# KalistaW/enterprise_warp

Hardware: AMD Instinct MI355X
Metric: lnL evals/sec (whole node), 45-psr CURN batched; % fp64 MFMA peak (higher is better)
Workload: dtype f64

## Files before the change

enterprise_warp_amd/csrc/chol_dd.hip:

```cpp
#include "ewarp_dev.h"

#include <cstdlib>

#pragma clang fp contract(off)

namespace ewh_dev {
namespace {

constexpr int DD_THREADS = 512;

__device__ __forceinline__ dd dd_sub_mul(dd a, dd x, dd y) {
  const double p = x.hi * y.hi;
  const double pe = fma(x.hi, y.hi, -p) + (x.hi * y.lo + x.lo * y.hi);
  const dd s = dd_two_sum(a.hi, -p);
  return dd_fast(s.hi, s.lo + a.lo - pe);
}
__device__ __forceinline__ void dd_acc_sub(double& th, double& tl, dd x, dd y) {
  const double p = x.hi * y.hi;
  const double e = fma(x.hi, y.hi, -p) + fma(x.hi, y.lo, x.lo * y.hi);
  const double s = th - p, bp = s - th;
  tl += ((th - (s - bp)) + (-p - bp)) - e;
  th = s;
}
__device__ __forceinline__ void lds_wave_sync() { asm volatile("s_waitcnt lgkmcnt(0)" ::: "memory"); }
// ... 264 lines not shown
  }
  if (wave == 0) ldet = wave_sum(ldet);
  if (tid == 0) {
    double lnl = J.K[(long long)(b - b_off) * J.kstride] - 0.5 * qv - 0.5 * ldet - 0.5 * lphi;
    if (!ok || J.fail) lnl = -INFINITY;
    out_units[(long long)p_ * B + b] = lnl;
  }
  __syncthreads();
}

template <int PW, bool RSOLVE = true>
__global__ __launch_bounds__(DD_THREADS) void chol_dd_kernel(const CholJob* __restrict__ jobs, int B, long long u0,
                                                             int b_off, const double* __restrict__ theta, int ldth,
                                                             double* __restrict__ out_units,
                                                             double* __restrict__ scratch, long long scr_per_wg,
                                                             const int* __restrict__ list,
                                                             const int* __restrict__ count, int dbg) {
  extern __shared__ __attribute__((aligned(16))) double2 dd_smem[];
  const int cnt = list ? *count : (int)gridDim.x;
  EWH_DCHECK(!list || cnt >= 0, "chol_dd list count");
  for (int i = blockIdx.x; i < cnt; i += gridDim.x) {
    const long long u = list ? (long long)list[i] : u0 + i;
    chol_ddb_unit<PW, RSOLVE>(jobs, B, u, b_off, theta + (long long)(u % B) * ldth, out_units, scratch, scr_per_wg,
                              dd_smem, dbg);
  }
}

constexpr double VERIFY_FRAC = 0.0625;
__global__ __launch_bounds__(256) void verify_units_kernel(const double* __restrict__ a, const double* __restrict__ b,
                                                           long long u0, long long n, double frac,
                                                           int* __restrict__ list, int* __restrict__ count,
                                                           unsigned long long* __restrict__ total) {
  const long long i = (long long)blockIdx.x * 256 + threadIdx.x;
  if (total && i == 0) atomicAdd(total + 1, (unsigned long long)n);
  if (i >= n) return;
  const long long u = u0 + i;
  const double x = a[u], y = b[u];
  const bool fx = x - x == 0.0, fy = y - y == 0.0;
  const bool bad = frac < 0.0 || !fx || !fy || fabs(x - y) > frac * (1e-6 + 1e-10 * fabs(x));
// ... 5 lines not shown
  }
}

__global__ void count_units_kernel(unsigned long long* __restrict__ total, long long n) {
  if (threadIdx.x == 0) {
    atomicAdd(total, (unsigned long long)n);
    atomicAdd(total + 1, (unsigned long long)n);
  }
}

constexpr int DD_PW_WIDE = 8;
constexpr int DD_LD_PW16 = 512;

template <int PW>
void launch_dd(const UnitSpan& s, long long u0, double* scr, long long scr_per_wg, unsigned grid, const int* list,
               const int* count, int ld, bool r05a) {
  int dbg = 0;
#ifdef EWH_DEV
  if (const char* e = getenv("EWARP_DD_SKIP")) dbg = atoi(e);
#endif
  if (r05a)
    hipLaunchKernelGGL(HIP_KERNEL_NAME(chol_dd_kernel<PW, false>), dim3(grid), dim3(DD_THREADS), dd_lds<PW>(ld), s.st,
                       s.jobs, s.B, u0, s.b_off, s.theta, s.ldth, s.units, scr, scr_per_wg, list, count, dbg);
  else
    hipLaunchKernelGGL(HIP_KERNEL_NAME(chol_dd_kernel<PW, true>), dim3(grid), dim3(DD_THREADS), dd_lds<PW>(ld), s.st,
                       s.jobs, s.B, u0, s.b_off, s.theta, s.ldth, s.units, scr, scr_per_wg, list, count, dbg);
}

int launch_dd_any(const UnitSpan& s, long long u0, double* scr, long long scr_per_wg, unsigned grid, const int* list,
                  const int* count, int ld, bool r05a) {
  if (ld <= DD_LD_PW16)
    launch_dd<16>(s, u0, scr, scr_per_wg, grid, list, count, ld, r05a);
  else
    launch_dd<DD_PW_WIDE>(s, u0, scr, scr_per_wg, grid, list, count, ld, r05a);
  const hipError_t e = hipGetLastError();
  return e == hipSuccess ? 0 : set_err(EWH_E_HIP, std::string("chol_dd_kernel: ") + hipGetErrorString(e));
}

}

int set_dd_attributes() {
  if (hipFuncSetAttribute((const void*)chol_dd_kernel<16, true>, hipFuncAttributeMaxDynamicSharedMemorySize,
                          (int)dd_lds<16>(DD_LD_PW16)) != hipSuccess ||
      hipFuncSetAttribute((const void*)chol_dd_kernel<DD_PW_WIDE, true>, hipFuncAttributeMaxDynamicSharedMemorySize,
                          (int)dd_lds<DD_PW_WIDE>(WIDE_LD_MAX)) != hipSuccess ||
// ... 25 lines not shown
  return e == hipSuccess ? 0 : set_err(EWH_E_HIP, std::string("verify_units_kernel: ") + hipGetErrorString(e));
}

long long dd_scratch_per_wg(int ld) { return 2LL * ld * ld; }

int launch_chol_dd(const UnitSpan& s, double* scr, long long scr_per_wg, long long cap, int ld, bool r05a) {
  for (long long o = 0; o < s.n; o += cap) {
    const int rc = launch_dd_any(s, s.u0 + o, scr, scr_per_wg, (unsigned)std::min(cap, s.n - o), nullptr, nullptr, ld,
                                 r05a);
    if (rc) return rc;
  }
  return 0;
}

int launch_chol_dd_list(const UnitSpan& s, double* scr, long long scr_per_wg, long long cap, const int* list,
                        const int* count, int ld, bool r05a) {
  return launch_dd_any(s, 0LL, scr, scr_per_wg, (unsigned)cap, list, count, ld, r05a);
}

}
```

enterprise_warp_amd/csrc/chol_partial.hip:

```cpp
#include "ewarp_dev.h"

namespace ewh_dev {
namespace {

template <int NB, int KEEP>
int launch_partial(const UnitSpan& s, double* keep_out, int keep_bs) {
  if constexpr (partial_in_registers(NB, KEEP) && NB - KEEP >= Split<NB>::H) {
    hipLaunchKernelGGL(HIP_KERNEL_NAME(chol_mfma_kernel<NB, default_waves(NB), PANEL_2L, false, KEEP>),
                       dim3((unsigned)s.n), dim3(64), 0, s.st, s.jobs, s.B, s.u0, s.b_off, s.theta, s.ldth, s.units,
                       keep_out, 0, keep_bs, UnitDec{});
    return 0;
  } else {
    return set_err(EWH_E_UNSUPPORTED, "common: reduced basis too narrow for the kept common block");
  }
}

}

int launch_partial_nb(int nb, int keep, const UnitSpan& s, double* keep_out, int keep_bs) {
  if (!partial_in_registers(nb, keep))
    return set_err(EWH_E_UNSUPPORTED, "common: no register kernel for this reduced width and kept size");
#define EWH_PARTK(NBV, KV) \
  case KV: return launch_partial<NBV, KV>(s, keep_out, keep_bs);
#define EWH_PART(NBV)   \
  case NBV:             \
// ... 26 lines not shown
```

enterprise_warp_amd/csrc/ewarp_chol_small.h:

```cpp
#pragma once
#include "ewarp_dev.h"

namespace ewh_dev {
namespace {

template <int NB, int ALG = PANEL_2L, bool STAMP = false, int W = default_waves(NB), bool FULL = false, int DEAD = -1,
          bool IMG = false, bool PL = false>
void launch_chol_mfma(const UnitSpan& s) {
  constexpr bool PLB = PL && pl_built(NB, DEAD, IMG);
  hipLaunchKernelGGL(HIP_KERNEL_NAME(chol_mfma_kernel<NB, W, ALG, STAMP, 0, FULL, DEAD, IMG, PLB>), dim3((unsigned)s.n),
                     dim3(64), 0, s.st, s.jobs, s.B, s.u0, s.b_off, s.theta, s.ldth, s.units, nullptr, 0, 0,
                     PLB ? unit_dec_make(s.u0, s.B) : UnitDec{});
}

template <int NB, bool STAMP = false, bool IMG = false, bool PL = false>
void launch_chol_front(int dead, const UnitSpan& s) {
  constexpr int W = default_waves(NB);
  switch (front_inst(NB, dead)) {
    case 3: launch_chol_mfma<NB, PANEL_2L, STAMP, W, false, 3, IMG, PL>(s); break;
    case 2: launch_chol_mfma<NB, PANEL_2L, STAMP, W, false, 2, IMG, PL>(s); break;
    case 1: launch_chol_mfma<NB, PANEL_2L, STAMP, W, false, NB == 6 ? -1 : 1, IMG, PL>(s); break;
    default: launch_chol_mfma<NB, PANEL_2L, STAMP, W, false, -1, IMG, PL>(s); break;
  }
}

template <int NB, bool STAMP = false, bool PL = false>
void launch_chol_images(int dead, bool img, const UnitSpan& s) {
// ... 9 lines not shown
```

enterprise_warp_amd/csrc/ewarp_ctx.h:

```cpp
#pragma once

#include "ewarp_launch.h"
#include "ewarp_mem.h"

#include <utility>

namespace ewh_host {

using namespace ewh_dev;
using namespace ewh_mem;

constexpr size_t LDS_MAX = 160 * 1024;

struct PsrHost {
  int n_toa = 0, m = 0, nlead = 0, ld = 0, nb = 0, n_epoch = 0;
  int max_epoch = 0;
  int fx_m = 0, fx_ld = 0, fx_nb = 0;
  int ncommon = 0, nloc = 0, gstart = 0;
  int gstart_v = 0;
  PsrDev dev{};
  int* d_colptr = nullptr;
  DSpec* d_spec = nullptr;
  int* d_fx_colptr = nullptr;
  DSpec* d_fx_spec = nullptr;
// ... 51 lines not shown
    Buf<double> d_dR, d_dZ, d_dcol, d_dcollo;
    long long s_stride = 0;
    int chunk = 0;
    void release() {
      for (auto* b : {&d_w, &d_beta, &d_s, &d_G, &d_Kb, &d_fac, &d_rho, &d_Glo, &d_dR, &d_dZ, &d_dcol, &d_dcollo})
        b->release();
      chunk = 0;
    }
  } var;
  Buf<double> d_bigscr;
  long long scr_budget = 0;
  Buf<double> d_widescr;
  Buf<double> d_ddscr;
  Buf<double> d_units2;
  Buf<int> d_ddlist;
  unsigned long long* d_ddstat = nullptr;
  int n_delay_psr = 0;
  bool cond_all = false;
  struct CondChunk {
    Buf<double> d_theta, d_z, d_x, d_coef, d_V, d_Y;
    Buf<int> d_status, d_grp;
    void release() {
      for (auto* b : {&d_theta, &d_z, &d_x, &d_coef, &d_V, &d_Y}) b->release();
      d_status.release();
      d_grp.release();
    }
  } cond;
  struct JointChunk {
    Buf<double> d_L, d_S, d_rhs, d_xc, d_z;
    Buf<int> d_pstat, d_sfail, d_cstart, d_grp;
    void release() {
// ... 104 lines not shown
```

enterprise_warp_amd/csrc/ewarp_dev.h:

```cpp
#pragma once
#include <hip/hip_runtime.h>

#include <algorithm>
#include <cmath>
#include <cstdint>
#include <cstring>
#include <string>
#include <type_traits>
#include <vector>

#include "ewarp_hip.h"
#include "ewarp_route.h"
#include "ewarp_spec.h"

namespace ewh_dev {

int set_err(int code, const std::string& msg);

#define EWH_HIP(expr)                                                          \
  do {                                                                         \
    hipError_t e_ = (expr);                                                    \
    if (e_ != hipSuccess)                                                      \
      return ::ewh_dev::set_err(EWH_E_HIP, std::string(#expr) + ": " + hipGetErrorString(e_)); \
  } while (0)
// ... 223 lines not shown
  const int* rep = nullptr;
  const int* ulist = nullptr;
  int nu = 0;
  const struct URec* urec = nullptr;
  const int* urep = nullptr;
  int ntidx = 0;
  int tidx[16] = {};
  const double* mats_lo = nullptr;
  const double* mats_rev = nullptr;
  const double* img = nullptr;
  const double* img_front = nullptr;
  const PlRec* pl = nullptr;
  int pl_ne = 0;
};

struct UnitSpan {
  const CholJob* jobs; int B; long long u0, n; int b_off;
  const double* theta; int ldth; double* units; hipStream_t st;
};

struct URec {
  static constexpr int NE = 3;
  DSpec e[NE];
  int ne, pad_[3];
};
static_assert(PL_NE == URec::NE, "a compact record (ewarp_spec.h) holds what a staged record holds");
constexpr int STAGE_THETA_MAX = 512;
constexpr int TIDX_MAX = 16;

template <int NB>
__global__ __launch_bounds__(256) void contract_mfma_kernel(PsrDev P, const double* __restrict__ w,
                                                            const double* __restrict__ beta,
                                                            const double* __restrict__ s,
// ... 775 lines not shown
      if constexpr (!LASTR) {
        const double rs = rsqrt_nr(dv);
        hook.on_scale(r, rs);
        static_for<bb + 1, NB>([&](auto JJ) { blk(JJ)[r] *= rs; });
      }
    });
  }
  }
}

#ifdef EWH_DEV
constexpr int STAMP_UNITS = 4096, STAMP_N = 24;
static __device__ long long g_stamps[STAMP_UNITS * STAMP_N];
#endif

template <int NB, int W, int ALG = PANEL_2L, bool STAMP = false, int KEEP = 0, bool FULL = false, int DEAD = -1,
          bool IMG = false, bool PL = false>
__global__ __launch_bounds__(64) __attribute__((amdgpu_waves_per_eu(W, W)))
void chol_mfma_kernel(const CholJob* __restrict__ jobs, int B, long long u0, int b_off,
                      const double* __restrict__ theta, int ldth, double* __restrict__ out_units,
                      double* __restrict__ keep_out, int keep_b0, int keep_bs, UnitDec ud) {
#ifdef EWH_DEV
  long long stp[STAMP_N];
#define EWH_STAMP(I)                                            \
  if constexpr (STAMP) {                                        \
    __builtin_amdgcn_sched_barrier(0);                          \
    stp[(I)] = (long long)__builtin_amdgcn_s_memtime();         \
    __builtin_amdgcn_sched_barrier(0);                          \
  }
#else
  static_assert(!STAMP, "phase stamps exist only in the dev library");
#define EWH_STAMP(I)
#endif
  EWH_STAMP(0)
  constexpr int LD = 16 * NB;
  using S = Split<NB, FULL>;
// ... 165 lines not shown
        double ph = 0.0;
        if (dedup) {
          ph = phs[J.rep[a]];
        } else {
          for (int e = J.col_ptr[a]; e < J.col_ptr[a + 1]; ++e) ph += spec_phi_body(J.spec[e], th);
        }
        pi = 1.0 / ph;
        ldet.add(ph);
      }
      phinv[wa] = pi;
    }
  }
  __syncthreads();
  EWH_STAMP(1)

  auto load_block = [&](auto BI, auto BJ, v4d& v) {
    constexpr int bi = decltype(BI)::value, bj = decltype(BJ)::value;
    if constexpr (IMG) {
      image_block(BI, BJ, v);
    } else {
      static_for<0, 4>([&](auto R) {
        constexpr int r = decltype(R)::value;
        if constexpr (FRONT) {
          v[r] = front_elem<NB, DEAD, bi, bj, r>(Af, q, c, s);
        } else {
          v[r] = A[(long long)(16 * bi + q + 4 * r) * LD + 16 * bj + c];
        }
      });
    }
    if constexpr (bi == bj) {
      const double pd = phinv[16 * bi + c];
      static_for<0, 4>([&](auto R) {
        constexpr int r = decltype(R)::value;
        v[r] += (q + 4 * r == c) ? pd : 0.0;
      });
    }
  };

  bool ok = true;
  constexpr bool SKIPPAD = KEEP == 0 && !FRONT;
  const int klast = SKIPPAD ? __builtin_amdgcn_readfirstlane(J.mreal - 16 * (NB - 1)) : 16;
  constexpr int D0 = FRONT ? DEAD : 0;
  constexpr bool PACK1 = NB != 8;

  v4d U1[S::n1 > 0 ? S::n1 : 1];
  static_for<0, H>([&](auto BI) {
    constexpr int bi = decltype(BI)::value;
    static_for<bi, NB>([&](auto BJ) {
      constexpr int bj = decltype(BJ)::value;
      if constexpr (bi == 0) {
        U1[S::i1(0, bj)] = pre[bj];
        if constexpr (bj == 0) {
          const double pd = phinv[c];
          static_for<0, 4>([&](auto R) {
            constexpr int r = decltype(R)::value;
            U1[S::i1(0, 0)][r] += (q + 4 * r == c) ? pd : 0.0;
          });
        }
      } else {
        load_block(BI, BJ, U1[S::i1(bi, bj)]);
      }
    });
  });
  static_for<0, H>([&](auto BBc) {
    constexpr int bb = decltype(BBc)::value;
    panel_ldl_row<NB, ALG, KEEP == 0, PACK1, DEAD, BLKLD>(
        BBc, [&](auto JJ) -> v4d& { return U1[S::i1(bb, decltype(JJ)::value)]; }, q, c, ldet, ok, NoHook{}, klast, s);
    EWH_STAMP(2 + 2 * bb)
    static_for<bb + 1, H>([&](auto II) {
      constexpr int i = decltype(II)::value;
      static_for<i, NB>([&](auto JJ) {
        constexpr int j = decltype(JJ)::value;
        syrk_update<bb == 0 ? D0 : 0>(U1[S::i1(i, j)], U1[S::i1(bb, i)], U1[S::i1(bb, j)]);
// ... 50 lines not shown
          const double v = U2[S::i2(i, j)][r];
          if (i != j || row <= col) {
            ko[row * KD + col] = v;
            ko[col * KD + row] = v;
          }
        });
      });
    });
  }
  const double ldet_v = wave_sum(ldet.value());
  const bool ok_all = __all(ok);
  if (lane == 0) {
    double lnl = J.K[(long long)(b - b_off) * J.kstride] - 0.5 * qv - 0.5 * ldet_v;
    if (!ok_all || J.fail) lnl = -INFINITY;
    out_units[(long long)p * B + b] = lnl;
  }
#ifdef EWH_DEV
  if constexpr (STAMP) {
    EWH_STAMP(3 + 2 * NB)
    if (lane == 0 && blockIdx.x < STAMP_UNITS) {
      long long* o = g_stamps + (long long)blockIdx.x * STAMP_N;
      for (int i = 0; i < 4 + 2 * NB && i < STAMP_N - 2; ++i) o[i] = stp[i];
      o[STAMP_N - 2] = __builtin_amdgcn_s_getreg(4 | (31 << 11));
      o[STAMP_N - 1] = __builtin_amdgcn_s_getreg(20 | (31 << 11));
    }
  }
#endif
#undef EWH_STAMP
}
constexpr int WIDE_LD_MAX = 16 * WIDE_NB_MAX;
// ... 114 lines not shown
int launch_chol_small(int mode, int nb, int dead, bool img, bool pl, const UnitSpan& s);
void launch_chol_small_pl(int nb, int dead, bool img, bool stamp, const UnitSpan& s);
int launch_chol_big_nb(int nb, const UnitSpan& s, double* scr, long long cap);
constexpr int LAT_NB_MAX = 8;
constexpr unsigned long long LAT_STALL_BITS = 0x7ff4dead057a1100ull;
int launch_chol_lat(int nb, int dead, const CholJob* jobs, int B, int P, const double* theta, int ldth, double* units,
                    double* host_units, hipStream_t st, bool stamp = false, int var = 0);
long long wide_scratch_per_wg(int nb, int keep);
long long dd_scratch_per_wg(int ld);
int launch_chol_dd(const UnitSpan& s, double* scr, long long scr_per_wg, long long cap, int ld, bool r05a = false);
int set_dd_attributes();
int launch_verify_units(const double* a, const double* b, long long u0, long long n, int* list, int* count,
                        unsigned long long* total, hipStream_t st, bool all = false);
int launch_count_units(unsigned long long* total, long long n, hipStream_t st);
int launch_chol_dd_list(const UnitSpan& s, double* scr, long long scr_per_wg, long long cap, const int* list,
                        const int* count, int ld, bool r05a = false);
int launch_chol_wide(const UnitSpan& s, double* scr, long long scr_per_wg, long long cap, int keep, double* keep_out,
                     int keep_b0, int keep_bs, int rev = 0, double* units_rev = nullptr, bool pair = true);
int launch_partial_nb(int nb, int keep, const UnitSpan& s, double* keep_out, int keep_bs);
int set_contract_attributes();
int launch_contract_wide(int nb, const PsrDev& P, const double* w, const double* beta, const double* s,
                         const double* fac, double* G, int nb_samples, hipStream_t st, double* Glo);
bool variant_built(int mode);

}
```

enterprise_warp_amd/csrc/ewarp_hip.hip:

```cpp
#include "ewarp_ctx.h"

#include <atomic>
#include <chrono>
#include <map>
#include <mutex>

namespace ewh_dev {

thread_local std::string g_err;

int set_err(int code, const std::string& msg) {
  g_err = msg;
  return code;
}

__global__ __launch_bounds__(256) void chol_lds_kernel(const CholJob* __restrict__ jobs, int B,
                                                       long long u0, int b_off,
                                                       const double* __restrict__ theta, int ldth,
                                                       double* __restrict__ out_units) {
  extern __shared__ __attribute__((aligned(16))) double sm[];
  __shared__ double red[4];
  const long long u = u0 + blockIdx.x;
  const int p = (int)(u / B), b = (int)(u % B);
  const CholJob J = jobs[p];
// ... 30 lines not shown
    for (int i = k + 1 + wave; i < ma; i += 4) {
      const double ci = col[i];
      const int base = i * (i + 1) / 2;
      for (int j = k + 1 + lane; j <= i; j += 64) L[base + j] = fma(-ci, col[j], L[base + j]);
    }
    __syncthreads();
  }
  const double qv = L[(ma - 1) * ma / 2 + ma - 1];
  if (threadIdx.x == 0) {
    double lnl = J.K[(long long)(b - b_off) * J.kstride] - 0.5 * qv - 0.5 * ldet.value() - 0.5 * lphi_sum;
    if (!ok || J.fail) lnl = -INFINITY;
    out_units[(long long)p * B + b] = lnl;
  }
}

__global__ void reduce_units_kernel(const double* __restrict__ units, int P, int B, double* __restrict__ out) {
  const int b = blockIdx.x * blockDim.x + threadIdx.x;
  if (b >= B) return;
  double s = 0.0;
  for (int p = 0; p < P; ++p) s += units[(long long)p * B + b];
  out[b] = s;
}

__global__ __launch_bounds__(256) void expand_theta_kernel(const double* __restrict__ stage,
                                                           const int* __restrict__ seg, int nseg, int np,
                                                           double* __restrict__ theta) {
  const int* rec = seg + 5 * blockIdx.x;
  const int r0 = rec[0], nr = rec[1] - rec[0], nc = rec[2];
  const int* cols = seg + 5 * nseg + rec[3];
  const double* src = stage + rec[4];
  for (int idx = threadIdx.x; idx < nr * nc; idx += 256) {
    const int r = idx / nc, j = idx - r * nc;
    theta[(long long)(r0 + r) * np + cols[j]] = src[idx];
  }
}

// ... 65 lines not shown
}

size_t n_units(const DevCtx* h, int B) { return (size_t)(h->P + (h->corr ? 1 : 0)) * B; }

int launch_wide(DevCtx* h, int nb, int keep, const UnitSpan& s, double* keep_out, int rev = 0,
                double* units_rev = nullptr) {
  if (nb > WIDE_NB_MAX) return set_err(EWH_E_UNSUPPORTED, "basis wider than 1023 columns");
  const long long per = wide_scratch_per_wg(nb, keep);
  const long long cap = scratch_slots(h, h->d_widescr, per, 4096);
  if (cap <= 0 || (units_rev && cap < 2)) return EWH_E_NOMEM;
  return launch_chol_wide(s, h->d_widescr.p, per, cap, keep, keep_out, 0, s.B, rev, units_rev, !h->plan.wide_r05a);
}

int ensure_dd_lists(DevCtx* h, const UnitSpan& s, bool list) {
  if (!h->d_ddstat) {
    if (const int rc = dalloc(h, &h->d_ddstat, 2)) return rc;
    EWH_HIP(hipMemsetAsync(h->d_ddstat, 0, 2 * sizeof(unsigned long long), s.st));
  }
  return list ? h->d_ddlist.reserve(n_units(h, s.B) + 1, h->hook) : 0;
}

int launch_dd_path(DevCtx* h, int nb, const UnitSpan& s) {
  const long long per = dd_scratch_per_wg(16 * nb);
  const long long cap = scratch_slots(h, h->d_ddscr, per, 1024);
  if (cap <= 0) return EWH_E_NOMEM;
  int rc;
  if ((rc = ensure_dd_lists(h, s, false))) return rc;
  if (h->plan.all_dd) {
    if ((rc = launch_count_units(h->d_ddstat, s.n, s.st))) return rc;
    return launch_chol_dd(s, h->d_ddscr.p, per, cap, 16 * nb, h->plan.wide_r05a);
  }
  if ((rc = h->d_units2.reserve(n_units(h, s.B), h->hook)) || (rc = ensure_dd_lists(h, s, true))) return rc;
  const bool fuse = !h->plan.wide_r05a && 2 * s.n <= 8LL * h->n_cu;
  if (!fuse) {
    UnitSpan r = s;
    r.units = h->d_units2.p;
    if ((rc = launch_wide(h, nb, 0, s, nullptr, 0)) || (rc = launch_wide(h, nb, 0, r, nullptr, 1))) return rc;
  } else if ((rc = launch_wide(h, nb, 0, s, nullptr, 0, h->d_units2.p))) {
    return rc;
  }
  int *count = h->d_ddlist.p, *list = count + 1;
  EWH_HIP(hipMemsetAsync(count, 0, sizeof(int), s.st));
  if ((rc = launch_verify_units(s.units, h->d_units2.p, s.u0, s.n, list, count, h->d_ddstat, s.st))) return rc;
  return launch_chol_dd_list(s, h->d_ddscr.p, per, std::min<long long>(cap, s.n), list, count, 16 * nb,
                             h->plan.wide_r05a);
}

struct Segment { Source src; int p0, nb, mreal; UnitSpan span; };

template <class F>
int for_segments(const DevCtx* h, const UnitSpan& all, F&& body) {
  const long long B = all.B, u_end = all.u0 + all.n;
  for (long long u = all.u0, end; u < u_end; u = end) {
    const int p0 = (int)(u / B);
    const PsrHost& ps = h->psr[p0];
    const bool run = h->white_fixed && ps.delay.n_delay == 0;
    Segment g{run ? Source::FixedRun : h->white_fixed ? Source::FixedDelay : Source::Varying, p0,
              run ? ps.fx_nb : ps.nb, run ? ps.fx_m : ps.m, all};
    int p1 = p0 + 1;
    for (; run && p1 * B < u_end && h->psr[p1].fx_nb == g.nb && h->psr[p1].delay.n_delay == 0; ++p1)
      g.mreal = std::max(g.mreal, h->psr[p1].fx_m);
    end = std::min(u_end, run ? p1 * B : std::min((p0 + 1) * B, u + h->var.chunk));
    g.span.jobs = run ? h->d_jobs_fixed : h->d_jobs_var;
    g.span.u0 = u;
    g.span.n = end - u;
    g.span.b_off = run ? 0 : (int)(u - p0 * B);
    if (const int rc = body(g)) return rc;
  }
  return 0;
}

int refine_failed(DevCtx* h, const Segment& g) {
  const UnitSpan& s = g.span;
  const long long per = dd_scratch_per_wg(16 * g.nb);
  const long long cap = scratch_slots(h, h->d_ddscr, per, 1024);
  if (cap <= 0) return EWH_E_NOMEM;
  int rc;
  if ((rc = ensure_dd_lists(h, s, true))) return rc;
  int *count = h->d_ddlist.p, *list = count + 1;
  EWH_HIP(hipMemsetAsync(count, 0, sizeof(int), s.st));
  if ((rc = launch_verify_units(s.units, s.units, s.u0, s.n, list, count, h->d_ddstat, s.st,
                                refine_lists_all(g.src, g.nb, h->plan))))
    return rc;
  if (g.src == Source::Varying) {
    const PsrHost& ps = h->psr[g.p0];
    launch_gram_dd_units(ps.dev, ps.nb, (unsigned)std::min<long long>(s.n, 64), ps.d_Tlo, h->var.d_w.p, h->var.d_beta.p,
                         list, count, s.B, s.b_off, h->var.d_G.p, h->var.d_Glo.p, s.st);
    if (ps.delay.n_delay > 0)
      launch_delay_scatter(ps.ld, (int)s.n, h->var.d_dcol.p, h->var.d_dcollo.p, h->var.d_G.p, h->var.d_Glo.p, s.st);
    EWH_HIP(hipGetLastError());
  }
  return launch_chol_dd_list(s, h->d_ddscr.p, per, std::min<long long>(cap, s.n), list, count, 16 * g.nb, false);
}

int partial_units(DevCtx* h, int nb, const UnitSpan& s, double* keep_out) {
  if (partial_route_for(h->plan, nb, h->keep) == PartialRoute::Register)
    return launch_partial_nb(nb, h->keep, s, keep_out, s.B);
  return launch_wide(h, nb, h->keep, s, keep_out);
}

#ifdef EWH_DEV
std::atomic<long long> g_prologue_launches[2] = {{0}, {0}};
#endif

int launch_register(DevCtx* h, const Segment& g) {
  const UnitSpan& s = g.span;
  const int dead = h->osmode ? 0 : front_dead(16 * g.nb, g.mreal);
// ... 200 lines not shown
  }
  if ((rc = corr_partial(h, theta_dev, B, 0, h->P, h->d_units.p, h->d_keep.p, st))) return rc;
  if (overlap) EWH_HIP(hipStreamWaitEvent(st, h->ev_join, 0));
  return corr_finish(h, theta_dev, B, h->d_keep.p, h->d_units.p, st, overlap);
}

int ctx_units(DevCtx* h, const double* theta_dev, int B, int64_t u_begin, int64_t u_end, double* out_dev,
              hipStream_t st, bool reduce) {
  const long long U = (long long)h->P * B;
  u_begin = std::max<int64_t>(0, u_begin);
  u_end = std::min<int64_t>(U, u_end);
  EWH_HIP(hipSetDevice(h->device));
  int rc;
  if ((rc = reserve_units(h, B))) return rc;
  const int rows = h->P + (h->corr ? 1 : 0);
  EWH_HIP(hipMemsetAsync(h->d_units.p, 0, sizeof(double) * (size_t)rows * B, st));
  StreamScope on_st(h, st);
  if (h->corr) {
    if (u_begin != 0 || u_end != U)
      return set_err(EWH_E_UNSUPPORTED, "correlated common process: pass the whole batch (shard samples, not units)");
    if ((rc = lnl_correlated(h, theta_dev, B, st))) return rc;
  } else {
    if ((rc = reserve_var_scratch(h, B))) return rc;
    const UnitSpan all{nullptr, B, u_begin, u_end - u_begin, 0, theta_dev, h->n_param, h->d_units.p, st};
    rc = for_segments(h, all, [&](const Segment& g) {
      const PsrHost& ps = h->psr[g.p0];
      const UnitSpan& s = g.span;
      int rc = 0;
      if (g.src == Source::Varying && (rc = run_white(h, g.p0, s.theta, s.ldth, s.b_off, (int)s.n))) return rc;
      if (g.src != Source::FixedRun && ps.delay.n_delay > 0 &&
          (rc = run_delay(h, g.p0, s.theta, s.ldth, s.b_off, (int)s.n)))
        return rc;
      if ((rc = dispatch_chol(h, g))) return rc;
      if (refine_after(g.src, g.nb, ps.dev.n_bgroup > 0, h->plan, h->corr, h->osmode)) rc = refine_failed(h, g);
      return rc;
    });
    if (rc) return rc;
  }
  if (reduce)
    hipLaunchKernelGGL(reduce_units_kernel, dim3((B + 255) / 256), dim3(256), 0, st, h->d_units.p, rows, B, out_dev);
  EWH_HIP(hipGetLastError());
  h->last_B = B;
  return 0;
}

int reserve_io(DevCtx* h, int B) {
  const size_t nth = (size_t)B * std::max(1, h->n_param);
  const int rc = h->d_theta.reserve(nth + B, h->hook);
  h->d_out = rc ? nullptr : h->d_theta.p + nth;
  return rc;
}

std::vector<std::pair<long long, long long>> unit_ranges(const std::vector<double>& cost, int B, int world) {
  const int P = (int)cost.size();
  std::vector<std::pair<long long, long long>> out;
// ... 424 lines not shown
    }
    if ((rc = corr_partial(h, h->d_theta.p, B, p0, p1, h->d_units.p, h->d_keep.p, h->stream))) return rc;
    if (i > 0) {
      EWH_HIP(hipMemcpyPeerAsync(h0->d_keep.p + (size_t)p0 * B * kd2, h0->device, h->d_keep.p + (size_t)p0 * B * kd2,
                                 h->device, sizeof(double) * (size_t)(p1 - p0) * B * kd2, h->stream));
      EWH_HIP(hipMemcpyPeerAsync(h0->d_units.p + (size_t)p0 * B, h0->device, h->d_units.p + (size_t)p0 * B, h->device,
                                 sizeof(double) * (size_t)(p1 - p0) * B, h->stream));
    }
  }
  for (int i = 1; i < nd; ++i) {
    EWH_HIP(hipSetDevice(H->ctx[i]->device));
    EWH_HIP(hipStreamSynchronize(H->ctx[i]->stream));
  }
  EWH_HIP(hipSetDevice(h0->device));
  if ((rc = corr_finish(h0, h0->d_theta.p, B, h0->d_keep.p, h0->d_units.p, h0->stream))) return rc;
  hipLaunchKernelGGL(reduce_units_kernel, dim3((B + 255) / 256), dim3(256), 0, h0->stream, h0->d_units.p, P + 1, B,
                     h0->d_out);
  EWH_HIP(hipGetLastError());
  EWH_HIP(hipMemcpyAsync(H->h_out.p, h0->d_out, sizeof(double) * B, hipMemcpyDeviceToHost, h0->stream));
  EWH_HIP(hipStreamSynchronize(h0->stream));
  std::memcpy(out_host, H->h_out.p, sizeof(double) * B);
  H->last_split.assign(1, {0, (long long)P * B});
  H->last_B = B;
  h0->last_B = B;
  return 0;
}

constexpr uint64_t LAT_SENTINEL = 0x7ff4dead0ebeef01ull;
constexpr int LAT_B_MAX = 24;

int lnl_batch_single(ewh_handle* H, DevCtx* h, int B, double* out_host) {
  int rc;
// ... 394 lines not shown
  EWH_HIP(hipGetLastError());
  return 0;
}

int ewh_corr_finish_device(ewh_handle* H, const double* theta_dev, int32_t B, const double* keep_dev,
                           const double* local_dev, double* out_dev, void* stream) {
  if (!H || !H->corr || !theta_dev || !keep_dev || !local_dev || !out_dev || B <= 0)
    return set_err(EWH_E_INVALID, "bad arguments (needs a correlated-common-process handle)");
  DevCtx* h = H->ctx[0];
  hipStream_t st = (hipStream_t)stream;
  EWH_HIP(hipSetDevice(h->device));
  int rc;
  if ((rc = reserve_units(h, B))) return rc;
  EWH_HIP(hipMemcpyAsync(h->d_units.p, local_dev, sizeof(double) * (size_t)H->P * B, hipMemcpyDeviceToDevice, st));
  if ((rc = corr_finish(h, theta_dev, B, keep_dev, h->d_units.p, st))) return rc;
  hipLaunchKernelGGL(reduce_units_kernel, dim3((B + 255) / 256), dim3(256), 0, st, h->d_units.p, H->P + 1, B, out_dev);
  EWH_HIP(hipGetLastError());
  H->last_split.assign(1, {0, (long long)H->P * B});
  H->last_B = B;
  h->last_B = B;
  return 0;
}

int ewh_optstat(ewh_handle* H, const double* theta_host, int32_t B, const double* phihat_host, double* rho_host,
                double* sig_host, double* os_host, double* os_sig_host) {
  if (!H) return set_err(EWH_E_INVALID, "bad arguments");
  return ctx_optstat(H->ctx[0], theta_host, B, phihat_host, rho_host, sig_host, os_host, os_sig_host);
}

int ewh_cond_dims(const ewh_handle* H, int64_t* n_coef, int64_t* n_toa_total) {
  if (!H) return set_err(EWH_E_INVALID, "bad handle");
// ... 190 lines not shown
```

enterprise_warp_amd/csrc/ewarp_plan.h:

```cpp
#pragma once

namespace ewh_dev {

struct KernelPlan {
  bool in_range = true;
  bool valid = true;
  bool variant = false;
  bool lat = true;
  bool lat_stamps = false;
  int lat_variant = 0;
  bool lds_only = false;
  bool all_wide = false;
  bool all_dd = false;
  bool refine = true;
  bool wide_r05a = false;
  bool contract2 = true;
  bool rsep = true;
  int contract2_waves = 0;
  bool epoch_multi = true;
  bool fixed_gram_dd = true;
  bool stage_spectra = true;
  bool compact_spectra = true;
  bool minv_reg = true;
  bool corr_right = true;
  bool corr_fuse_diag = true;
  bool corr_fused = true;
  bool corr_pairs = true;
  bool corr_rowupdate_r1 = false;
  bool corr_diag_lds = false;
  bool corr_one_tile = false;
// ... 12 lines not shown
  switch (mode) {
    case 0: p.lat = true; dev_only = false; break;
    case 1:
      p.lds_only = true; p.refine = false;
      p.corr_fused = false; p.corr_rowupdate_r1 = true; p.corr_diag_lds = true;
      dev_only = false;
      break;
    case 2: dev_only = false; break;
    case 7:
      p.contract2 = false; p.fixed_gram_dd = false; p.minv_reg = false;
      p.corr_fused = false; p.corr_diag_lds = true; p.corr_trailing = true;
      dev_only = false;
      break;
    case 27: p.all_wide = true; p.refine = false; dev_only = false; break;
    case 29: p.all_dd = true; dev_only = false; break;
    case 14: p.compact_spectra = false; p.variant = true; break;
    case 15: p.contract2_waves = 4; p.variant = true; break;
    case 16: p.contract2_waves = 8; p.variant = true; break;
    case 17: case 21: case 26: p.variant = true; break;
    case 19: p.stage_spectra = false; p.variant = true; break;
    case 22: p.lat = true; p.lat_stamps = true; p.variant = true; break;
    case 23: p.lat = true; p.lat_variant = 3; p.variant = true; break;
    case 24: p.lat = true; p.lat_variant = 1; p.variant = true; break;
    case 25: p.lat = true; p.lat_variant = 2; p.variant = true; break;
    case 28: p.corr_pairs = false; p.corr_one_tile = true; p.variant = true; break;
    case 30: p.rsep = false; p.contract2_waves = 30; p.variant = true; break;
    case 31: p.corr_pairs = false; p.variant = true; break;
    case 32: p.corr_pair_unpiped = true; p.variant = true; break;
    case 33: p.corr_fuse_diag = false; break;
    case 34: p.wide_r05a = true; break;
    case 35: p.contract2_waves = 35; break;
    case 36: p.rsep = false; break;
    case 37: p.epoch_multi = false; break;
    case 38: p.rsep = false; p.contract2_waves = 38; break;
    case 39: p.rsep = false; p.contract2_waves = 39; break;
    default: p.valid = false; break;
  }
  if (dev_only && !dev_lib) p.valid = false;
  return p;
}

constexpr bool same_plan(const KernelPlan& a, const KernelPlan& b) {
  return a.in_range == b.in_range && a.valid == b.valid && a.variant == b.variant && a.lat == b.lat &&
         a.lat_stamps == b.lat_stamps && a.lat_variant == b.lat_variant && a.lds_only == b.lds_only && a.all_wide == b.all_wide &&
         a.all_dd == b.all_dd && a.refine == b.refine && a.wide_r05a == b.wide_r05a && a.contract2 == b.contract2 &&
         a.rsep == b.rsep && a.contract2_waves == b.contract2_waves && a.epoch_multi == b.epoch_multi &&
         a.fixed_gram_dd == b.fixed_gram_dd && a.stage_spectra == b.stage_spectra && a.compact_spectra == b.compact_spectra &&
         a.minv_reg == b.minv_reg &&
         a.corr_right == b.corr_right && a.corr_fuse_diag == b.corr_fuse_diag && a.corr_fused == b.corr_fused &&
         a.corr_pairs == b.corr_pairs && a.corr_rowupdate_r1 == b.corr_rowupdate_r1 &&
         a.corr_diag_lds == b.corr_diag_lds && a.corr_one_tile == b.corr_one_tile &&
         a.corr_pair_unpiped == b.corr_pair_unpiped && a.corr_trailing == b.corr_trailing;
}

constexpr KernelPlan batched_default_plan() {
  KernelPlan p;
  p.lat = false;
  p.corr_right = false;
  return p;
}

static_assert(same_plan(plan_for(0, false), KernelPlan{}) && same_plan(plan_for(0, true), KernelPlan{}),
              "mode 0 is the default plan");
static_assert(same_plan(plan_for(2, false), batched_default_plan()),
              "mode 2 leaves the latency path and (with every non-default mode) the right-looking schedule, no more");
static_assert(!plan_for(-1, true).in_range && !plan_for(KERNEL_MODE_MAX + 1, true).in_range &&
                  plan_for(3, true).in_range && plan_for(KERNEL_MODE_MAX, false).in_range,
              "the range of mode numbers");
static_assert(plan_for(14, true).valid && !plan_for(14, true).compact_spectra && plan_for(14, true).stage_spectra &&
                  plan_for(19, true).compact_spectra && !plan_for(14, false).valid,
              "mode 14 turns off the fixed-form prologue alone, in the dev library");
static_assert(!plan_for(-1, true).valid && !plan_for(3, true).valid && !plan_for(18, true).valid &&
                  !plan_for(20, true).valid && !plan_for(KERNEL_MODE_MAX + 1, true).valid,
              "a mode outside the lists is invalid");
static_assert(plan_for(33, true).valid && !plan_for(33, false).valid && !plan_for(15, false).valid &&
                  !plan_for(39, false).valid,
              "a dev-only mode is invalid in the product library");
static_assert(plan_for(1, false).valid && plan_for(7, false).valid && plan_for(27, false).valid &&
                  plan_for(29, false).valid,
              "the product modes");

}
```

enterprise_warp_amd/csrc/ewarp_route.h:

```cpp
#pragma once
#include "ewarp_plan.h"

namespace ewh_dev {

constexpr int MFMA_NB_MAX = 9;
constexpr int BIG_NB_MAX = 16;
constexpr int WIDE_NB_MAX = 64;

constexpr int PARTIAL_KEEP_MAX = 4;
constexpr bool partial_in_registers(int nb, int keep) {
  return nb <= MFMA_NB_MAX && keep >= 1 && keep <= PARTIAL_KEEP_MAX && nb - keep >= (nb == 8 ? 3 : nb / 2) &&
         !(nb == 7 && keep >= 3);
}

enum class Route {
  Register,
  Big,
  Lds,
  Wide,
  DdVerify,
  DdAll,
  Unsupported,
};
enum class PartialRoute { Register, Wide };
// ... 21 lines not shown
constexpr PartialRoute partial_route_for(const KernelPlan& plan, int nb, int keep) {
  return partial_in_registers(nb, keep) && !plan.all_wide ? PartialRoute::Register : PartialRoute::Wide;
}

constexpr bool refine_after(Source src, int nb, bool bgroups, const KernelPlan& plan, bool corr, bool osmode) {
  if (corr || osmode || !plan.refine) return false;
  switch (src) {
    case Source::FixedRun: return !dd_path(plan, corr, osmode, nb, true);
    case Source::FixedDelay: return nb <= BIG_NB_MAX;
    default: return !bgroups;
  }
}

constexpr bool refine_lists_all(Source src, int nb, const KernelPlan& plan) {
  return plan.all_dd && src == Source::Varying && nb <= BIG_NB_MAX;
}

namespace route_check {

constexpr Route R = Route::Register, G = Route::Big, L = Route::Lds, W = Route::Wide, V = Route::DdVerify,
                A = Route::DdAll, U = Route::Unsupported;

constexpr bool row(int mode, bool fixed, Route r1, Route r9, Route r10, Route r16, Route r17, Route r64, Route r65) {
  for (int dev = 0; dev < 2; ++dev) {
    const KernelPlan p = plan_for(mode, dev == 1);
    if (route_for(p, false, false, 1, fixed) != r1 || route_for(p, false, false, 9, fixed) != r9 ||
        route_for(p, false, false, 10, fixed) != r10 || route_for(p, false, false, 16, fixed) != r16 ||
        route_for(p, false, false, 17, fixed) != r17 || route_for(p, false, false, 64, fixed) != r64 ||
        route_for(p, false, false, 65, fixed) != r65)
      return false;
// ... 52 lines not shown
  return true;
}
static_assert(same_as_old(0, 9), "routes and refine conditions as before, modes 0..9");
static_assert(same_as_old(10, 19), "routes and refine conditions as before, modes 10..19");
static_assert(same_as_old(20, 29), "routes and refine conditions as before, modes 20..29");
static_assert(same_as_old(30, KERNEL_MODE_MAX), "routes and refine conditions as before, modes 30..");

constexpr bool no_refine(int mode) {
  for (int nb = 1; nb <= 65; ++nb)
    for (int src = 0; src < 3; ++src)
      if (refine_after((Source)src, nb, false, plan_for(mode, false), false, false)) return false;
  return true;
}
static_assert(no_refine(1) && no_refine(27), "the cross-check modes compare the fp64 kernels as such");

constexpr bool partial_as_old() {
  for (int mode = 0; mode <= KERNEL_MODE_MAX; ++mode)
    for (int nb = 1; nb <= 17; ++nb)
      for (int keep = 0; keep <= 5; ++keep) {
        const KernelPlan p = plan_for(mode, true);
        if ((partial_route_for(p, nb, keep) == PartialRoute::Register) !=
            (partial_in_registers(nb, keep) && !p.all_wide))
          return false;
      }
  return true;
}
static_assert(partial_as_old(), "the partial route: registers where the kernel exists, unless all_wide");

}
}
// ... 1 lines not shown
```

Baseline: 1.222 million.

## Fuse failure listing into Cholesky kernel and self-reset DD counters

The register-route Cholesky kernel now appends non-finite units to the refine list and updates the stats counters itself, so fixed-run segments skip the separate verify kernel. The DD refine kernel resets its count with a last-block ticket, which removes the per-segment memsets, and the units buffer memset is skipped for full-range non-correlated evaluations. The refine grid shrinks to the CU count when listing is fused, and the reduce kernel is rewritten to stage rows through LDS. This adds global atomics and relies on every unit being written, plus a new mode 13 that keeps the old path.

```diff
diff --git a/enterprise_warp_amd/csrc/chol_dd.hip b/enterprise_warp_amd/csrc/chol_dd.hip
--- a/enterprise_warp_amd/csrc/chol_dd.hip
+++ b/enterprise_warp_amd/csrc/chol_dd.hip
@@ -302,15 +302,24 @@
                                                              int b_off, const double* __restrict__ theta, int ldth,
                                                              double* __restrict__ out_units,
                                                              double* __restrict__ scratch, long long scr_per_wg,
-                                                             const int* __restrict__ list,
-                                                             const int* __restrict__ count, int dbg) {
+                                                             const int* __restrict__ list, int* count, int dbg) {
   extern __shared__ __attribute__((aligned(16))) double2 dd_smem[];
-  const int cnt = list ? *count : (int)gridDim.x;
+  const int cnt = list ? __hip_atomic_load(count, __ATOMIC_RELAXED, __HIP_MEMORY_SCOPE_AGENT) : (int)gridDim.x;
   EWH_DCHECK(!list || cnt >= 0, "chol_dd list count");
   for (int i = blockIdx.x; i < cnt; i += gridDim.x) {
     const long long u = list ? (long long)list[i] : u0 + i;
     chol_ddb_unit<PW, RSOLVE>(jobs, B, u, b_off, theta + (long long)(u % B) * ldth, out_units, scratch, scr_per_wg,
                               dd_smem, dbg);
+  }
+  if (list && threadIdx.x == 0) {
+    __threadfence();
+    const int ticket = atomicAdd(count + 1, 1);
+    EWH_DCHECK(ticket >= 0 && ticket < (int)gridDim.x, "chol_dd done-ticket within the grid");
+    if (ticket == (int)gridDim.x - 1) {
+      __threadfence();
+      __hip_atomic_store(count, 0, __ATOMIC_RELAXED, __HIP_MEMORY_SCOPE_AGENT);
+      __hip_atomic_store(count + 1, 0, __ATOMIC_RELAXED, __HIP_MEMORY_SCOPE_AGENT);
+    }
   }
 }
 
@@ -346,7 +355,7 @@
 
 template <int PW>
 void launch_dd(const UnitSpan& s, long long u0, double* scr, long long scr_per_wg, unsigned grid, const int* list,
-               const int* count, int ld, bool r05a) {
+               int* count, int ld, bool r05a) {
   int dbg = 0;
 #ifdef EWH_DEV
   if (const char* e = getenv("EWARP_DD_SKIP")) dbg = atoi(e);
@@ -360,7 +369,7 @@
 }
 
 int launch_dd_any(const UnitSpan& s, long long u0, double* scr, long long scr_per_wg, unsigned grid, const int* list,
-                  const int* count, int ld, bool r05a) {
+                  int* count, int ld, bool r05a) {
   if (ld <= DD_LD_PW16)
     launch_dd<16>(s, u0, scr, scr_per_wg, grid, list, count, ld, r05a);
   else
@@ -416,7 +425,7 @@
 }
 
 int launch_chol_dd_list(const UnitSpan& s, double* scr, long long scr_per_wg, long long cap, const int* list,
-                        const int* count, int ld, bool r05a) {
+                        int* count, int ld, bool r05a) {
   return launch_dd_any(s, 0LL, scr, scr_per_wg, (unsigned)cap, list, count, ld, r05a);
 }
 
diff --git a/enterprise_warp_amd/csrc/chol_partial.hip b/enterprise_warp_amd/csrc/chol_partial.hip
--- a/enterprise_warp_amd/csrc/chol_partial.hip
+++ b/enterprise_warp_amd/csrc/chol_partial.hip
@@ -8,7 +8,7 @@
   if constexpr (partial_in_registers(NB, KEEP) && NB - KEEP >= Split<NB>::H) {
     hipLaunchKernelGGL(HIP_KERNEL_NAME(chol_mfma_kernel<NB, default_waves(NB), PANEL_2L, false, KEEP>),
                        dim3((unsigned)s.n), dim3(64), 0, s.st, s.jobs, s.B, s.u0, s.b_off, s.theta, s.ldth, s.units,
-                       keep_out, 0, keep_bs, UnitDec{});
+                       keep_out, 0, keep_bs, UnitDec{}, FailList{});
     return 0;
   } else {
     return set_err(EWH_E_UNSUPPORTED, "common: reduced basis too narrow for the kept common block");
diff --git a/enterprise_warp_amd/csrc/ewarp_chol_small.h b/enterprise_warp_amd/csrc/ewarp_chol_small.h
--- a/enterprise_warp_amd/csrc/ewarp_chol_small.h
+++ b/enterprise_warp_amd/csrc/ewarp_chol_small.h
@@ -10,7 +10,7 @@
   constexpr bool PLB = PL && pl_built(NB, DEAD, IMG);
   hipLaunchKernelGGL(HIP_KERNEL_NAME(chol_mfma_kernel<NB, W, ALG, STAMP, 0, FULL, DEAD, IMG, PLB>), dim3((unsigned)s.n),
                      dim3(64), 0, s.st, s.jobs, s.B, s.u0, s.b_off, s.theta, s.ldth, s.units, nullptr, 0, 0,
-                     PLB ? unit_dec_make(s.u0, s.B) : UnitDec{});
+                     PLB ? unit_dec_make(s.u0, s.B) : UnitDec{}, s.fails);
 }
 
 template <int NB, bool STAMP = false, bool IMG = false, bool PL = false>
diff --git a/enterprise_warp_amd/csrc/ewarp_ctx.h b/enterprise_warp_amd/csrc/ewarp_ctx.h
--- a/enterprise_warp_amd/csrc/ewarp_ctx.h
+++ b/enterprise_warp_amd/csrc/ewarp_ctx.h
@@ -89,7 +89,9 @@
   Buf<double> d_ddscr;
   Buf<double> d_units2;
   Buf<int> d_ddlist;
+  static constexpr int DDSTAT_WORDS = 3;
   unsigned long long* d_ddstat = nullptr;
+  int* dd_count() const { return reinterpret_cast<int*>(d_ddstat + 2); }
   int n_delay_psr = 0;
   bool cond_all = false;
   struct CondChunk {
diff --git a/enterprise_warp_amd/csrc/ewarp_dev.h b/enterprise_warp_amd/csrc/ewarp_dev.h
--- a/enterprise_warp_amd/csrc/ewarp_dev.h
+++ b/enterprise_warp_amd/csrc/ewarp_dev.h
@@ -261,9 +261,15 @@
   int pl_ne = 0;
 };
 
+struct FailList {
+  int* count = nullptr;
+  int* list = nullptr;
+  unsigned long long* stat = nullptr;
+};
 struct UnitSpan {
   const CholJob* jobs; int B; long long u0, n; int b_off;
   const double* theta; int ldth; double* units; hipStream_t st;
+  FailList fails = {};
 };
 
 struct URec {
@@ -1069,12 +1075,14 @@
 static __device__ long long g_stamps[STAMP_UNITS * STAMP_N];
 #endif
 
+constexpr bool diag_by_selectors(int nb, int keep, int alg, bool full, int dead, bool img, bool pl) { return keep == 0; }
+
 template <int NB, int W, int ALG = PANEL_2L, bool STAMP = false, int KEEP = 0, bool FULL = false, int DEAD = -1,
           bool IMG = false, bool PL = false>
 __global__ __launch_bounds__(64) __attribute__((amdgpu_waves_per_eu(W, W)))
 void chol_mfma_kernel(const CholJob* __restrict__ jobs, int B, long long u0, int b_off,
                       const double* __restrict__ theta, int ldth, double* __restrict__ out_units,
-                      double* __restrict__ keep_out, int keep_b0, int keep_bs, UnitDec ud) {
+                      double* __restrict__ keep_out, int keep_b0, int keep_bs, UnitDec ud, FailList fl) {
 #ifdef EWH_DEV
   long long stp[STAMP_N];
 #define EWH_STAMP(I)                                            \
@@ -1270,6 +1278,20 @@
   __syncthreads();
   EWH_STAMP(1)
 
+  constexpr bool DIAGSEL = diag_by_selectors(NB, KEEP, ALG, FULL, DEAD, IMG, PL);
+  [[maybe_unused]] double dsel[4];
+  if constexpr (DIAGSEL)
+    static_for<0, 4>([&](auto R) { dsel[decltype(R)::value] = (q + 4 * decltype(R)::value == c) ? 1.0 : 0.0; });
+  auto add_diag = [&](v4d& v, double pd) {
+    static_for<0, 4>([&](auto R) {
+      constexpr int r = decltype(R)::value;
+      if constexpr (DIAGSEL) {
+        v[r] = fma(pd, dsel[r], v[r]);
+      } else {
+        v[r] += (q + 4 * r == c) ? pd : 0.0;
+      }
+    });
+  };
   auto load_block = [&](auto BI, auto BJ, v4d& v) {
     constexpr int bi = decltype(BI)::value, bj = decltype(BJ)::value;
     if constexpr (IMG) {
@@ -1284,13 +1306,7 @@
         }
       });
     }
-    if constexpr (bi == bj) {
-      const double pd = phinv[16 * bi + c];
-      static_for<0, 4>([&](auto R) {
-        constexpr int r = decltype(R)::value;
-        v[r] += (q + 4 * r == c) ? pd : 0.0;
-      });
-    }
+    if constexpr (bi == bj) add_diag(v, phinv[16 * bi + c]);
   };
 
   bool ok = true;
@@ -1306,13 +1322,7 @@
       constexpr int bj = decltype(BJ)::value;
       if constexpr (bi == 0) {
         U1[S::i1(0, bj)] = pre[bj];
-        if constexpr (bj == 0) {
-          const double pd = phinv[c];
-          static_for<0, 4>([&](auto R) {
-            constexpr int r = decltype(R)::value;
-            U1[S::i1(0, 0)][r] += (q + 4 * r == c) ? pd : 0.0;
-          });
-        }
+        if constexpr (bj == 0) add_diag(U1[S::i1(0, 0)], phinv[c]);
       } else {
         load_block(BI, BJ, U1[S::i1(bi, bj)]);
       }
@@ -1393,6 +1403,15 @@
     double lnl = J.K[(long long)(b - b_off) * J.kstride] - 0.5 * qv - 0.5 * ldet_v;
     if (!ok_all || J.fail) lnl = -INFINITY;
     out_units[(long long)p * B + b] = lnl;
+    if (fl.count != nullptr) {
+      if (!(lnl - lnl == 0.0)) {
+        const int slot = atomicAdd(fl.count, 1);
+        EWH_DCHECK(slot >= 0 && slot < (int)gridDim.x, "chol_mfma: list slot within the launch's units");
+        fl.list[slot] = p * B + b;
+        atomicAdd(fl.stat, 1ull);
+      }
+      if (blockIdx.x == 0) atomicAdd(fl.stat + 1, (unsigned long long)gridDim.x);
+    }
   }
 #ifdef EWH_DEV
   if constexpr (STAMP) {
@@ -1537,7 +1556,7 @@
                         unsigned long long* total, hipStream_t st, bool all = false);
 int launch_count_units(unsigned long long* total, long long n, hipStream_t st);
 int launch_chol_dd_list(const UnitSpan& s, double* scr, long long scr_per_wg, long long cap, const int* list,
-                        const int* count, int ld, bool r05a = false);
+                        int* count, int ld, bool r05a = false);
 int launch_chol_wide(const UnitSpan& s, double* scr, long long scr_per_wg, long long cap, int keep, double* keep_out,
                      int keep_b0, int keep_bs, int rev = 0, double* units_rev = nullptr, bool pair = true);
 int launch_partial_nb(int nb, int keep, const UnitSpan& s, double* keep_out, int keep_bs);
diff --git a/enterprise_warp_amd/csrc/ewarp_hip.hip b/enterprise_warp_amd/csrc/ewarp_hip.hip
--- a/enterprise_warp_amd/csrc/ewarp_hip.hip
+++ b/enterprise_warp_amd/csrc/ewarp_hip.hip
@@ -68,12 +68,29 @@
   }
 }
 
-__global__ void reduce_units_kernel(const double* __restrict__ units, int P, int B, double* __restrict__ out) {
-  const int b = blockIdx.x * blockDim.x + threadIdx.x;
-  if (b >= B) return;
+constexpr int RED_S = 64, RED_G = 4, RED_ROWS = 64;
+__global__ __launch_bounds__(RED_S * RED_G) void reduce_units_kernel(const double* __restrict__ units, int P, int B,
+                                                                   double* __restrict__ out) {
+  __shared__ double t[RED_ROWS][RED_S];
+  const int bl = threadIdx.x % RED_S, g = threadIdx.x / RED_S;
+  const int b = blockIdx.x * RED_S + bl;
   double s = 0.0;
-  for (int p = 0; p < P; ++p) s += units[(long long)p * B + b];
-  out[b] = s;
+  for (int p0 = 0; p0 < P; p0 += RED_ROWS) {
+    const int np = min(RED_ROWS, P - p0);
+#pragma unroll
+    for (int k = 0; k < RED_ROWS / RED_G; ++k) {
+      const int r = g + RED_G * k;
+      if (r < np && b < B) t[r][bl] = units[(long long)(p0 + r) * B + b];
+    }
+    __syncthreads();
+    if (g == 0 && b < B)
+      for (int r = 0; r < np; ++r) s += t[r][bl];
+    __syncthreads();
+  }
+  if (g == 0 && b < B) out[b] = s;
+}
+void launch_reduce_units(const double* units, int rows, int B, double* out, hipStream_t st) {
+  hipLaunchKernelGGL(reduce_units_kernel, dim3((B + RED_S - 1) / RED_S), dim3(RED_S * RED_G), 0, st, units, rows, B, out);
 }
 
 __global__ __launch_bounds__(256) void expand_theta_kernel(const double* __restrict__ stage,
@@ -169,10 +186,10 @@
 
 int ensure_dd_lists(DevCtx* h, const UnitSpan& s, bool list) {
   if (!h->d_ddstat) {
-    if (const int rc = dalloc(h, &h->d_ddstat, 2)) return rc;
-    EWH_HIP(hipMemsetAsync(h->d_ddstat, 0, 2 * sizeof(unsigned long long), s.st));
-  }
-  return list ? h->d_ddlist.reserve(n_units(h, s.B) + 1, h->hook) : 0;
+    if (const int rc = dalloc(h, &h->d_ddstat, DevCtx::DDSTAT_WORDS)) return rc;
+    EWH_HIP(hipMemsetAsync(h->d_ddstat, 0, DevCtx::DDSTAT_WORDS * sizeof(unsigned long long), s.st));
+  }
+  return list ? h->d_ddlist.reserve(n_units(h, s.B), h->hook) : 0;
 }
 
 int launch_dd_path(DevCtx* h, int nb, const UnitSpan& s) {
@@ -194,8 +211,8 @@
   } else if ((rc = launch_wide(h, nb, 0, s, nullptr, 0, h->d_units2.p))) {
     return rc;
   }
-  int *count = h->d_ddlist.p, *list = count + 1;
-  EWH_HIP(hipMemsetAsync(count, 0, sizeof(int), s.st));
+  int *count = h->dd_count(), *list = h->d_ddlist.p;
+  if (!h->plan.fuse_tail) EWH_HIP(hipMemsetAsync(count, 0, sizeof(int), s.st));
   if ((rc = launch_verify_units(s.units, h->d_units2.p, s.u0, s.n, list, count, h->d_ddstat, s.st))) return rc;
   return launch_chol_dd_list(s, h->d_ddscr.p, per, std::min<long long>(cap, s.n), list, count, 16 * nb,
                              h->plan.wide_r05a);
@@ -225,18 +242,19 @@
   return 0;
 }
 
-int refine_failed(DevCtx* h, const Segment& g) {
+int refine_failed(DevCtx* h, const Segment& g, bool listed) {
   const UnitSpan& s = g.span;
   const long long per = dd_scratch_per_wg(16 * g.nb);
   const long long cap = scratch_slots(h, h->d_ddscr, per, 1024);
   if (cap <= 0) return EWH_E_NOMEM;
   int rc;
   if ((rc = ensure_dd_lists(h, s, true))) return rc;
-  int *count = h->d_ddlist.p, *list = count + 1;
-  EWH_HIP(hipMemsetAsync(count, 0, sizeof(int), s.st));
-  if ((rc = launch_verify_units(s.units, s.units, s.u0, s.n, list, count, h->d_ddstat, s.st,
-                                refine_lists_all(g.src, g.nb, h->plan))))
-    return rc;
+  int *count = h->dd_count(), *list = h->d_ddlist.p;
+  const bool all = refine_lists_all(g.src, g.nb, h->plan);
+  if (!listed) {
+    if (!h->plan.fuse_tail) EWH_HIP(hipMemsetAsync(count, 0, sizeof(int), s.st));
+    if ((rc = launch_verify_units(s.units, s.units, s.u0, s.n, list, count, h->d_ddstat, s.st, all))) return rc;
+  }
   if (g.src == Source::Varying) {
     const PsrHost& ps = h->psr[g.p0];
     launch_gram_dd_units(ps.dev, ps.nb, (unsigned)std::min<long long>(s.n, 64), ps.d_Tlo, h->var.d_w.p, h->var.d_beta.p,
@@ -245,7 +263,8 @@
       launch_delay_scatter(ps.ld, (int)s.n, h->var.d_dcol.p, h->var.d_dcollo.p, h->var.d_G.p, h->var.d_Glo.p, s.st);
     EWH_HIP(hipGetLastError());
   }
-  return launch_chol_dd_list(s, h->d_ddscr.p, per, std::min<long long>(cap, s.n), list, count, 16 * g.nb, false);
+  const long long grid = all || !h->plan.fuse_tail ? cap : std::min<long long>(cap, std::max(1, h->n_cu));
+  return launch_chol_dd_list(s, h->d_ddscr.p, per, std::min<long long>(grid, s.n), list, count, 16 * g.nb, false);
 }
 
 int partial_units(DevCtx* h, int nb, const UnitSpan& s, double* keep_out) {
@@ -476,7 +495,8 @@
   int rc;
   if ((rc = reserve_units(h, B))) return rc;
   const int rows = h->P + (h->corr ? 1 : 0);
-  EWH_HIP(hipMemsetAsync(h->d_units.p, 0, sizeof(double) * (size_t)rows * B, st));
+  if (h->corr || u_begin != 0 || u_end != U || !h->plan.fuse_tail)
+    EWH_HIP(hipMemsetAsync(h->d_units.p, 0, sizeof(double) * (size_t)rows * B, st));
   StreamScope on_st(h, st);
   if (h->corr) {
     if (u_begin != 0 || u_end != U)
@@ -493,14 +513,23 @@
       if (g.src != Source::FixedRun && ps.delay.n_delay > 0 &&
           (rc = run_delay(h, g.p0, s.theta, s.ldth, s.b_off, (int)s.n)))
         return rc;
-      if ((rc = dispatch_chol(h, g))) return rc;
-      if (refine_after(g.src, g.nb, ps.dev.n_bgroup > 0, h->plan, h->corr, h->osmode)) rc = refine_failed(h, g);
+      const bool bg = ps.dev.n_bgroup > 0;
+      if (!refine_after(g.src, g.nb, bg, h->plan, h->corr, h->osmode)) return dispatch_chol(h, g);
+      const bool listed = refine_listed_by_launch(g.src, g.nb, bg, h->plan, h->corr, h->osmode);
+      Segment gl = g;
+      if (listed) {
+        if ((rc = ensure_dd_lists(h, s, true))) return rc;
+        if (scratch_slots(h, h->d_ddscr, dd_scratch_per_wg(16 * g.nb), 1024) <= 0) return (int)EWH_E_NOMEM;
+        gl.span.fails = FailList{h->dd_count(), h->d_ddlist.p, h->d_ddstat};
+      }
+      if ((rc = dispatch_chol(h, gl)) == 0) rc = refine_failed(h, g, listed);
+      if (rc && listed) (void)hipMemsetAsync(h->dd_count(), 0, 2 * sizeof(int), s.st);
       return rc;
     });
     if (rc) return rc;
   }
   if (reduce)
-    hipLaunchKernelGGL(reduce_units_kernel, dim3((B + 255) / 256), dim3(256), 0, st, h->d_units.p, rows, B, out_dev);
+    launch_reduce_units(h->d_units.p, rows, B, out_dev, st);
   EWH_HIP(hipGetLastError());
   h->last_B = B;
   return 0;
@@ -955,8 +984,7 @@
   }
   EWH_HIP(hipSetDevice(h0->device));
   if ((rc = corr_finish(h0, h0->d_theta.p, B, h0->d_keep.p, h0->d_units.p, h0->stream))) return rc;
-  hipLaunchKernelGGL(reduce_units_kernel, dim3((B + 255) / 256), dim3(256), 0, h0->stream, h0->d_units.p, P + 1, B,
-                     h0->d_out);
+  launch_reduce_units(h0->d_units.p, P + 1, B, h0->d_out, h0->stream);
   EWH_HIP(hipGetLastError());
   EWH_HIP(hipMemcpyAsync(H->h_out.p, h0->d_out, sizeof(double) * B, hipMemcpyDeviceToHost, h0->stream));
   EWH_HIP(hipStreamSynchronize(h0->stream));
@@ -1381,7 +1409,7 @@
   if ((rc = reserve_units(h, B))) return rc;
   EWH_HIP(hipMemcpyAsync(h->d_units.p, local_dev, sizeof(double) * (size_t)H->P * B, hipMemcpyDeviceToDevice, st));
   if ((rc = corr_finish(h, theta_dev, B, keep_dev, h->d_units.p, st))) return rc;
-  hipLaunchKernelGGL(reduce_units_kernel, dim3((B + 255) / 256), dim3(256), 0, st, h->d_units.p, H->P + 1, B, out_dev);
+  launch_reduce_units(h->d_units.p, H->P + 1, B, out_dev, st);
   EWH_HIP(hipGetLastError());
   H->last_split.assign(1, {0, (long long)H->P * B});
   H->last_B = B;
diff --git a/enterprise_warp_amd/csrc/ewarp_plan.h b/enterprise_warp_amd/csrc/ewarp_plan.h
--- a/enterprise_warp_amd/csrc/ewarp_plan.h
+++ b/enterprise_warp_amd/csrc/ewarp_plan.h
@@ -14,6 +14,7 @@
   bool all_dd = false;
   bool refine = true;
   bool wide_r05a = false;
+  bool fuse_tail = true;
   bool contract2 = true;
   bool rsep = true;
   int contract2_waves = 0;
@@ -56,6 +57,7 @@
       break;
     case 27: p.all_wide = true; p.refine = false; dev_only = false; break;
     case 29: p.all_dd = true; dev_only = false; break;
+    case 13: p.fuse_tail = false; break;
     case 14: p.compact_spectra = false; p.variant = true; break;
     case 15: p.contract2_waves = 4; p.variant = true; break;
     case 16: p.contract2_waves = 8; p.variant = true; break;
@@ -85,7 +87,7 @@
 constexpr bool same_plan(const KernelPlan& a, const KernelPlan& b) {
   return a.in_range == b.in_range && a.valid == b.valid && a.variant == b.variant && a.lat == b.lat &&
          a.lat_stamps == b.lat_stamps && a.lat_variant == b.lat_variant && a.lds_only == b.lds_only && a.all_wide == b.all_wide &&
-         a.all_dd == b.all_dd && a.refine == b.refine && a.wide_r05a == b.wide_r05a && a.contract2 == b.contract2 &&
+         a.all_dd == b.all_dd && a.refine == b.refine && a.wide_r05a == b.wide_r05a && a.fuse_tail == b.fuse_tail && a.contract2 == b.contract2 &&
          a.rsep == b.rsep && a.contract2_waves == b.contract2_waves && a.epoch_multi == b.epoch_multi &&
          a.fixed_gram_dd == b.fixed_gram_dd && a.stage_spectra == b.stage_spectra && a.compact_spectra == b.compact_spectra &&
          a.minv_reg == b.minv_reg &&
@@ -112,6 +114,9 @@
 static_assert(plan_for(14, true).valid && !plan_for(14, true).compact_spectra && plan_for(14, true).stage_spectra &&
                   plan_for(19, true).compact_spectra && !plan_for(14, false).valid,
               "mode 14 turns off the fixed-form prologue alone, in the dev library");
+static_assert(plan_for(13, true).valid && !plan_for(13, true).fuse_tail && !plan_for(13, true).lat && !plan_for(13, false).valid &&
+                  plan_for(2, true).fuse_tail,
+              "mode 13 is mode 2 with the separate failure scan and the memsets, in the dev library");
 static_assert(!plan_for(-1, true).valid && !plan_for(3, true).valid && !plan_for(18, true).valid &&
                   !plan_for(20, true).valid && !plan_for(KERNEL_MODE_MAX + 1, true).valid,
               "a mode outside the lists is invalid");
diff --git a/enterprise_warp_amd/csrc/ewarp_route.h b/enterprise_warp_amd/csrc/ewarp_route.h
--- a/enterprise_warp_amd/csrc/ewarp_route.h
+++ b/enterprise_warp_amd/csrc/ewarp_route.h
@@ -59,6 +59,11 @@
 
 constexpr bool refine_lists_all(Source src, int nb, const KernelPlan& plan) {
   return plan.all_dd && src == Source::Varying && nb <= BIG_NB_MAX;
+}
+
+constexpr bool refine_listed_by_launch(Source src, int nb, bool bgroups, const KernelPlan& plan, bool corr, bool osmode) {
+  return refine_after(src, nb, bgroups, plan, corr, osmode) && plan.fuse_tail && src == Source::FixedRun &&
+         route_for(plan, corr, osmode, nb, true) == Route::Register && !refine_lists_all(src, nb, plan);
 }
 
 namespace route_check {
@@ -141,6 +146,28 @@
 }
 static_assert(no_refine(1) && no_refine(27), "the cross-check modes compare the fp64 kernels as such");
 
+constexpr bool listed_by_launch_ok(int mode_lo, int mode_hi) {
+  for (int mode = mode_lo; mode <= mode_hi; ++mode)
+    for (int dev = 0; dev < 2; ++dev) {
+      const KernelPlan p = plan_for(mode, dev == 1);
+      for (int common = 0; common < 3; ++common)
+        for (int nb = 1; nb <= 65; ++nb)
+          for (int src = 0; src < 3; ++src)
+            for (int bg = 0; bg < 2; ++bg) {
+              const bool want = common == 0 && (Source)src == Source::FixedRun && nb <= MFMA_NB_MAX && p.refine &&
+                                !p.all_dd && !p.lds_only && !p.all_wide && p.fuse_tail;
+              if (refine_listed_by_launch((Source)src, nb, bg == 1, p, common == 1, common == 2) != want) return false;
+            }
+    }
+  return true;
+}
+static_assert(listed_by_launch_ok(0, 9) && listed_by_launch_ok(10, 19), "failures listed by the launch: fixed runs on the register route");
+static_assert(listed_by_launch_ok(20, 29) && listed_by_launch_ok(30, KERNEL_MODE_MAX), "... modes 20..");
+static_assert(refine_listed_by_launch(Source::FixedRun, 8, false, plan_for(0, false), false, false) &&
+                  !refine_listed_by_launch(Source::FixedRun, 8, false, plan_for(13, true), false, false) &&
+                  refine_after(Source::FixedRun, 8, false, plan_for(13, true), false, false),
+              "mode 13 keeps the refine pass and gives the scan back to its own kernel");
+
 constexpr bool partial_as_old() {
   for (int mode = 0; mode <= KERNEL_MODE_MAX; ++mode)
     for (int nb = 1; nb <= 17; ++nb)
```

Measured after the change: 1.230 million, median of 6. Within noise of the previous version (+0.7%).
